# DeepRank/Deeprank-GNN

Hardware: AMD Instinct MI355X
Metric: interface-graphs/sec (fwd+bwd) GINet batch=64 per GPU (higher is better)
Workload: dtype f32; 1 GPU; GINet train step (topology + body fwd + FC head/MSE + bwd + grad all-reduce + Adam) on SYN graphs: 200 nodes, ~1000 directed edges, 32 node feats, 50->16 clusters (BASELINE.json configs[1]); graphs_per_gpu=64, global_batch=64, parallelism=dp1, mode=native, step_layout=auto

## Files before the change

### deeprank-gnn_amd/csrc/drgnn_step.h

```cpp
#ifndef DRGNN_STEP_H
#define DRGNN_STEP_H

#include "drgnn_net.h"

#ifndef DRGNN_SKIP
#define DRGNN_SKIP (-1)
#endif
#define PH(k) if (DRGNN_SKIP != (k))
#ifndef DRGNN_EXIT_AFTER
#define DRGNN_EXIT_AFTER (-1)
#endif
#define EXIT_AFTER(k)                                                                          \
    do {                                                                                       \
        if (DRGNN_EXIT_AFTER == (k)) {                                                         \
            float acc_ = 0.0f;                                                                 \
            if ((k) > 0) { FOR_TID(i_, (int)(s.end - scratch)) { acc_ += scratch[i_]; } }      \
            if (acc_ == 12345.678f) a.hf.pred[0] = acc_;                                       \
            return;                                                                            \
        }                                                                                      \
    } while (0)

struct StepArgs {
    drgnn_net_desc net;
    const float* x;
// ... 59 lines not shown
    X(mem1, capC, 1)                                                                           \
    X(a0, ((long)capC * DRGNN_H1 + 1) / 2, 1)                                                    \
    X(a1, ((long)capC * DRGNN_H2 + 1) / 2, 1)                                                    \
    X(u1, (long)(capN + 4) * hc1, 1)                                                           \
    X(z1, (long)capN * DRGNN_H1, 1)                                                            \
    X(dv0, capN, !gin)                                                                         \
    X(sc0, capN, !gin)                                                                         \
    X(xp, (long)(capC + 4) * STEP_XPLD, 1)                                                     \
    X(u2, (long)(capC + 4) * (DRGNN_H2 + 4), 1)                                                \
    X(z2, (long)(capC + 4) * (DRGNN_H2 + 4), 1)                                                \
    X(p2, (gin ? ((long)capC * DRGNN_H2 > (long)(capC + 4) * STEP_XPLD ? (long)capC * DRGNN_H2 : (long)(capC + 4) * STEP_XPLD) \
               : (long)(capC + 4) * (DRGNN_H2 + 4)), 1)                                        \
    X(dv1, capC, !gin)                                                                         \
    X(sc1, capC, !gin)                                                                         \
    X(hw2, (long)O * H, 1)                                                                     \
    X(hb2, O, 1)

HD int64_t step_scratch_words(int kind, int64_t F, int64_t capN, int64_t capE, int64_t capC, int64_t R,
                              int64_t H, int64_t O) {
    const int64_t hc1 = (kind == DRGNN_GINET) ? DRGNN_H1 : 2 * DRGNN_H1;
    const int64_t hc2 = (kind == DRGNN_GINET) ? DRGNN_H2 : 2 * DRGNN_H2;
    const int sg = (kind == DRGNN_SGAT) ? 1 : 0;
    const int gin = (kind == DRGNN_GINET) ? 1 : 0;
    const int64_t xld = step_pad16((int)F) + 4;
    int64_t w = 0;
#define X(name, words, cond) w += (cond) ? (((int64_t)(words) + 3) & ~(int64_t)3) : 0;
    STEP_CARVE_LIST(X)
#undef X
    return w + 16;
}

#define STEP_M_BAD 0
#define STEP_M_Y 1
#define STEP_M_WY 2
#define STEP_M_DENOM 3
#define STEP_WB_J 4

static inline bool step_burst_guaranteed(int kind, const float* x, int F, int capN, int capE, int capC, int H, int O) {
    if (H != ((kind == DRGNN_GINET) ? 128 : 64)) return false;
    return ((((uintptr_t)x) & 15) == 0) && (F % 4 == 0) && (F * DRGNN_H1 <= DRGNN_BCAP) && ((long)capN * F <= 16L * DRGNN_BCAP) &&
           (capN + 1 <= DRGNN_BCAP) && (capE <= 2 * DRGNN_BCAP) && (capC * DRGNN_H1 <= 4 * DRGNN_BCAP) &&
           O * H <= 2 * DRGNN_BCAP && H * 8 <= STEP_WB_J * DRGNN_BCAP;
}

#define STEP_CLS_N 200
#define STEP_CLS_E 1024
#define STEP_CLS_C 52

#ifndef DRGNN_EMU
#define STEP_PIN(x) asm volatile("" : "+v"(x))


template <bool RELU = false>
DEV void step_gemm_nn(int M, int NT, int K, const float* A, int lda, const float* Bt, int ldbt, float* C, int ldc,
                      int* dummy, const float* bias = nullptr, const float* nan_rows = nullptr, int wave_shift = 0) {
    const int wave = (__builtin_amdgcn_readfirstlane((int)(threadIdx.x >> 6)) - wave_shift) & (DRGNN_NWAVES - 1);
    const int lane = threadIdx.x & 63;
    const int lr = lane & 15, lq = lane >> 4;
    const int units = ((M + 15) >> 4) * NT;
    for (int u = wave; u < units; u += DRGNN_NWAVES) {
        const int ti = (NT == 1) ? u : (u >> 1), tj = (NT == 1) ? 0 : (u & 1);
        const float* ap = A + (ti * 16 + lr) * lda + 4 * lq;
        const float* bp = Bt + (tj * 16 + lr) * ldbt + 4 * lq;
        drgnn_f32x4 acc = {0.f, 0.f, 0.f, 0.f};
        for (int k0 = 0; k0 < K; k0 += 32) {
            const drgnn_f4 a0 = *(const drgnn_f4*)(ap + k0), b0 = *(const drgnn_f4*)(bp + k0);
            const bool two = k0 + 16 < K;
            drgnn_f4 a1 = a0, b1 = b0;
            if (two) { a1 = *(const drgnn_f4*)(ap + k0 + 16); b1 = *(const drgnn_f4*)(bp + k0 + 16); }
#pragma unroll
            for (int j = 0; j < 4; ++j) acc = __builtin_amdgcn_mfma_f32_16x16x4f32(a0[j], b0[j], acc, 0, 0, 0);
            if (two) {
#pragma unroll
                for (int j = 0; j < 4; ++j) acc = __builtin_amdgcn_mfma_f32_16x16x4f32(a1[j], b1[j], acc, 0, 0, 0);
            }
        }
#pragma unroll
        for (int r = 0; r < 4; ++r) {
            const int ci = ti * 16 + lq * 4 + r;
            float* p = (ci < M) ? C + ci * ldc + tj * 16 + lr : (float*)dummy + lane;
            float v = acc[r];
            if (bias) v += bias[tj * 16 + lr];
            if (nan_rows && ci < M && nan_rows[ci] == 0.0f) v = DRGNN_NAN;
            if (RELU) v = (v < 0.0f) ? 0.0f : v;
            *p = v;
        }
    }
}

template <int LD, class IdxT>
DEV void step_gather_rows(int n, const int* rp, const IdxT* col, const float* src, float* dst) {
    const int items = ((n * 16) + 63) & ~63;
    for (int item = threadIdx.x; item < items; item += DRGNN_NTHREADS) {
        const int i = item >> 4, sl = (item >> 2) & 3, c = (item & 3) * 4;
        float a0 = 0.f, a1 = 0.f, a2 = 0.f, a3 = 0.f;
        if (i < n) {
            const int lo = rp[i], hi = rp[i + 1];
            for (int k = lo + sl; k < hi; k += 4) {
                const drgnn_f4 v = *(const drgnn_f4*)(src + ROW24(col[k], LD) + c);
                a0 += v[0]; a1 += v[1]; a2 += v[2]; a3 += v[3];
            }
        }
        a0 += dpp_take<0x128>(a0); a1 += dpp_take<0x128>(a1); a2 += dpp_take<0x128>(a2); a3 += dpp_take<0x128>(a3);
        a0 += dpp_take<0x124>(a0); a1 += dpp_take<0x124>(a1); a2 += dpp_take<0x124>(a2); a3 += dpp_take<0x124>(a3);
        if (sl == 0 && i < n) *(drgnn_f4*)(dst + i * LD + c) = drgnn_f4{a0, a1, a2, a3};
    }
}

DEV void xchg_publish(unsigned long long* slot, uint32_t tag, float v);
template <int LDZ, bool SKIP0 = false>
DEV void step_pool_readout(int C1, const int* mp, const int* mem, const float* z, short* arg, const float* misc,
                           float* xr, float* g_readout, const int* rp = nullptr, unsigned long long* pub = nullptr,
                           uint32_t tag = 0u, int a1ld = 0) {
    int bad; memcpy(&bad, &misc[STEP_M_BAD], 4);
    const float inv = 1.0f / (float)(C1 > 0 ? C1 : 1);
    for (int t = threadIdx.x; t < DRGNN_H2 * 16; t += DRGNN_NTHREADS) {
        const int c = t >> 4, kk = t & 15;
        float acc = 0.0f;
        for (int k = kk; k < C1; k += 16) {
            float best = DRGNN_NEG_INF;
            int am = -1;
            const int plo = mp[k], phi = mp[k + 1];
            for (int p = plo; p < phi; p += 4) {
                int mm[4];
                float vv[4];
#pragma unroll
                for (int j = 0; j < 4; ++j) mm[j] = mem[(p + j < phi) ? p + j : phi - 1];
#pragma unroll
                for (int j = 0; j < 4; ++j) {
                    vv[j] = z[ROW24(mm[j], LDZ) + c];
                    if (SKIP0 && rp[mm[j] + 1] == rp[mm[j]]) vv[j] = DRGNN_NAN;
                }
#pragma unroll
                for (int j = 0; j < 4; ++j)
                    if (vv[j] > best) { best = vv[j]; am = mm[j]; }
            }
            if (am < 0) best = 0.0f;
            arg[a1ld ? c * a1ld + k : k * DRGNN_H2 + c] = (short)((best > 0.0f) ? am : -1);
            acc += best;
        }
        acc = lanes16_sum(acc) * inv;
        if (bad) acc = DRGNN_NAN;
        if (kk == 0) {
            if (pub) xchg_publish(pub + c, tag, acc);
            xr[c] = acc; out_store(&g_readout[c], acc);
        }
    }
}

DEV void xchg_publish(unsigned long long* slot, uint32_t tag, float v) {
    const unsigned long long w = ((unsigned long long)tag << 32) | (unsigned long long)__float_as_uint(v);
    __hip_atomic_store(slot, w, __ATOMIC_RELAXED, __HIP_MEMORY_SCOPE_AGENT);
}
DEV float xchg_wait(unsigned long long* slot, uint32_t tag, int32_t* fault) {
    const unsigned long long t0 = wall_clock64();
    for (;;) {
        const unsigned long long w = __hip_atomic_load(slot, __ATOMIC_RELAXED, __HIP_MEMORY_SCOPE_AGENT);
        if ((uint32_t)(w >> 32) == tag) return __uint_as_float((uint32_t)w);
        if (wall_clock64() - t0 > 30000000ull) { atomicOr(fault, DRGNN_FAULT_EXCHANGE); return DRGNN_NAN; }
        __builtin_amdgcn_s_sleep(1);
    }
}
DEV unsigned long long xchg_peek(const unsigned long long* slot) {
    return __hip_atomic_load(slot, __ATOMIC_RELAXED, __HIP_MEMORY_SCOPE_AGENT);
}
DEV float xchg_finish(unsigned long long* slot, unsigned long long w, uint32_t tag, int32_t* fault) {
    if ((uint32_t)(w >> 32) == tag) return __uint_as_float((uint32_t)w);
    return xchg_wait(slot, tag, fault);
}

template <int WJ> struct WBlockRegs { drgnn_f4 v[WJ * DRGNN_BSCALE]; };
template <int WJ> DEV void step_wblock_load(WBlockRegs<WJ>& wr, const HeadFused& hf, int br) {
    const bool vec = ((((uintptr_t)hf.w1) & 15) == 0);
#pragma unroll
    for (int j = 0; j < WJ * DRGNN_BSCALE; ++j) {
        const int t = threadIdx.x + j * DRGNN_NTHREADS;
        const int h = t >> 3, q = t & 7;
        drgnn_f4 v = {0.f, 0.f, 0.f, 0.f};
        if (h < hf.H) {
            const float* src = hf.w1 + (long)h * hf.R + br * DRGNN_H2 + 4 * q;
            if (vec) v = *(const drgnn_f4*)src;
            else { v[0] = src[0]; v[1] = src[1]; v[2] = src[2]; v[3] = src[3]; }
        }
        wr.v[j] = v;
    }
}
template <int WJ> DEV void step_wblock_store(const WBlockRegs<WJ>& wr, const HeadFused& hf, int br, float* wb) {
    (void)br;
#pragma unroll
    for (int j = 0; j < WJ * DRGNN_BSCALE; ++j) {
        const int t = threadIdx.x + j * DRGNN_NTHREADS;
        const int h = t >> 3, q = t & 7;
        if (h < hf.H) *(drgnn_f4*)(wb + h * STEP_WBLD + 4 * q) = wr.v[j];
    }
}

template <int HC, int WJ>
DEV void step_head_fc1_t(const HeadFused& hf, int g, int br, int nb, const float* wb, const WBlockRegs<WJ>& wo,
                         const float* b1, const float* xr, float* hid, unsigned long long* xg, uint32_t tag, uint32_t step,
                         uint32_t thresh, float keep_scale, int32_t* fault) {
    const int H = HC ? HC : hf.H;
    const int lane = threadIdx.x & 63;
    unsigned long long* const slot = xg + (long)(1 - br) * DRGNN_H2 + (lane & (DRGNN_H2 - 1));
    unsigned long long w0 = 0ull;
    if (nb > 1 && lane < DRGNN_H2) w0 = xchg_peek(slot);
    const int items = (H * 8 + 63) & ~63;
    drgnn_f4 xo = {0.f, 0.f, 0.f, 0.f};
    bool have_other = false;
    int j = 0;
    for (int t = threadIdx.x; t < items; t += DRGNN_NTHREADS, ++j) {
        const int h = t >> 3, q = t & 7;
        float acc = 0.0f;
        if (h < H) {
            const drgnn_f4 w = *(const drgnn_f4*)(wb + h * STEP_WBLD + 4 * q);
            const drgnn_f4 x = *(const drgnn_f4*)(xr + 4 * q);
            acc = fmaf(w[0], x[0], fmaf(w[1], x[1], fmaf(w[2], x[2], w[3] * x[3])));
        }
        acc = lanes8_sum(acc);
        float v = acc;
        if (nb > 1) {
            if (!have_other) {
                float pv = 0.0f;
                PH(7) { if (lane < DRGNN_H2) pv = xchg_finish(slot, w0, tag, fault); }
                const int src = (lane & 7) * 4;
                xo[0] = __shfl(pv, src, 64); xo[1] = __shfl(pv, src + 1, 64);
                xo[2] = __shfl(pv, src + 2, 64); xo[3] = __shfl(pv, src + 3, 64);
                have_other = true;
            }
            float other = 0.0f;
            if (h < H) {
                const drgnn_f4 w = wo.v[j < WJ * DRGNN_BSCALE ? j : 0];
                other = fmaf(w[0], xo[0], fmaf(w[1], xo[1], fmaf(w[2], xo[2], w[3] * xo[3])));
            }
            other = lanes8_sum(other);
            v = (br == 0) ? acc + other : other + acc;
        }
        if (q == 0 && h < H) {
            v += b1[h];
            v = v > 0.0f ? v : 0.0f;
            if (thresh) v = drgnn_keep(hf, step, g, H, h, thresh) ? v * keep_scale : 0.0f;
            hid[h] = v;
        }
    }
}
template <int WREF, bool ONLY, int WJ>
DEV void step_head_fc1(const HeadFused& hf, int g, int br, int nb, const float* wb, const WBlockRegs<WJ>& wo, const float* b1,
                       const float* xr, float* hid, unsigned long long* xg, uint32_t tag, uint32_t step,
                       uint32_t thresh, float keep_scale, int32_t* fault) {
    if (ONLY || hf.H == WREF) step_head_fc1_t<WREF, WJ>(hf, g, br, nb, wb, wo, b1, xr, hid, xg, tag, step, thresh, keep_scale, fault);
    else step_head_fc1_t<0, WJ>(hf, g, br, nb, wb, wo, b1, xr, hid, xg, tag, step, thresh, keep_scale, fault);
}

template <int HC, int OC>
DEV void step_head_loss_t(const HeadFused& hf, int g, int br, const float* hid, const float* w2, const float* b2,
                          const float* misc, float keep_scale, float* dhid, float* p_dhid, float* p_hw2,
                          float* p_hb2, float* p_loss) {
    const int H = HC ? HC : hf.H, O = OC ? OC : hf.O;
    if (__builtin_expect(!hf.train, 0)) {
        if (br == 0) {
            FOR_TID(o, O) {
                float acc = b2[o];
                for (int h = 0; h < H; ++h) acc = fmaf(hid[h], w2[o * H + h], acc);
                if (hf.sigmoid && hf.task != DRGNN_TASK_CLASS) acc = drgnn_sigmoid(acc);
                out_store(&hf.pred[(long)g * O + o], acc);
            }
        }
        return;
    }
    const bool ext = hf.task == DRGNN_TASK_GRAD;
    const bool sig = hf.sigmoid && hf.task != DRGNN_TASK_CLASS;
    const float denom = misc[STEP_M_DENOM], wy = misc[STEP_M_WY];
    if ((int)(threadIdx.x & ~63u) >= H && threadIdx.x >= 64) return;
    const int lane = threadIdx.x & 63;
    if (HC != 0 && HC <= 128 && OC == 1 && hf.task != DRGNN_TASK_CLASS) {
        constexpr int NH = (HC > 0) ? (HC + 63) / 64 : 1;
        float hv[NH], wv[NH];
#pragma unroll
        for (int j = 0; j < NH; ++j) { hv[j] = hid[lane + 64 * j]; wv[j] = w2[lane + 64 * j]; }
        const float bias = b2[0], yv = misc[STEP_M_Y];
        float acc = 0.0f;
#pragma unroll
        for (int j = 0; j < NH; ++j) acc = fmaf(hv[j], wv[j], acc);
        float out = lanes64_sum(acc) + bias;
        if (sig) out = drgnn_sigmoid(out);
        const float inv = 1.0f / (float)(hf.B * O);
        const float d = out - yv;
        const float dout = (ext ? yv : 2.0f * d * inv) * (sig ? out * (1.0f - out) : 1.0f);
        const int wv_id = (int)(threadIdx.x >> 6);
        float hme = hv[0], wme = wv[0];
#pragma unroll
        for (int j = 1; j < NH; ++j) { if (wv_id == j) { hme = hv[j]; wme = wv[j]; } }
        const int h = (int)threadIdx.x;
        const float dh = (hme != 0.0f) ? fmaf(dout, wme, 0.0f) * keep_scale : 0.0f;
        dhid[h] = dh;
        if (br == 0) {
            out_store(&p_hw2[h], dout * hme);
            out_store(&p_dhid[h], dh);
            if (threadIdx.x == 0) {
                out_store(&hf.pred[(long)g], out);
                out_store(&p_hb2[0], dout);
                out_store(&p_loss[0], ext ? 0.0f : (d * d * inv));
                out_store(&p_loss[1], 1.0f);
            }
        }
        return;
    }
    float my_out = 0.0f;
    for (int o = 0; o < O; ++o) {
        float acc = 0.0f;
        for (int h = lane; h < H; h += 64) acc = fmaf(hid[h], w2[o * H + h], acc);
        acc = lanes64_sum(acc) + b2[o];
        if (lane == o) my_out = acc;
    }
    if (sig) my_out = drgnn_sigmoid(my_out);
    float my_dout = 0.0f, loss, wsum = 1.0f;
    if (ext) {
        loss = 0.0f;
        my_dout = lane < O ? hf.y_reg[(long)g * O + lane] * (sig ? my_out * (1.0f - my_out) : 1.0f) : 0.0f;
    } else if (__builtin_expect(hf.task == DRGNN_TASK_REG, 1)) {
        const float inv = 1.0f / (float)(hf.B * O);
        const float d = my_out - misc[STEP_M_Y];
        loss = lanes64_sum(lane < O ? d * d * inv : 0.0f);
        my_dout = lane < O ? 2.0f * d * inv * (sig ? my_out * (1.0f - my_out) : 1.0f) : 0.0f;
    } else {
        const int yc = __builtin_amdgcn_readfirstlane(__float_as_int(misc[STEP_M_Y]));
        const float mx = lanes64_max(lane < O ? my_out : DRGNN_NEG_INF);
        const float se = lanes64_sum(lane < O ? expf(my_out - mx) : 0.0f);
        const float lse = logf(se) + mx;
        loss = wy * (lse - lane_get(my_out, yc)) / denom;
        my_dout = lane < O ? wy * (expf(my_out - lse) - (lane == yc ? 1.0f : 0.0f)) / denom : 0.0f;
        wsum = wy;
    }
    if (br == 0 && (int)threadIdx.x < O) {
        out_store(&hf.pred[(long)g * O + threadIdx.x], my_out);
        out_store(&p_hb2[threadIdx.x], my_dout);
    }
    if (br == 0 && threadIdx.x == 0) { out_store(&p_loss[0], loss); out_store(&p_loss[1], wsum); }
    for (int h0 = 0; h0 < H; h0 += DRGNN_NTHREADS) {
        const int h = h0 + (int)threadIdx.x;
        const bool ok = h < H;
        const float hv = ok ? hid[h] : 0.0f;
        float acc = 0.0f;
        for (int o = 0; o < O; ++o) {
            const float dout = lane_get(my_dout, o);
            if (ok) {
                acc = fmaf(dout, w2[o * H + h], acc);
                if (br == 0) out_store(&p_hw2[(long)o * H + h], dout * hv);
            }
        }
        if (ok) {
            const float dh = (hv != 0.0f) ? acc * keep_scale : 0.0f;
            dhid[h] = dh;
            if (br == 0) out_store(&p_dhid[h], dh);
        }
    }
}
template <int WREF, bool ONLY>
DEV void step_head_loss(const HeadFused& hf, int g, int br, const float* hid, const float* w2, const float* b2,
                        const float* misc, float keep_scale, float* dhid, float* p_dhid, float* p_hw2,
                        float* p_hb2, float* p_loss) {
    if (__builtin_expect(hf.H == WREF && hf.O == 1, 1))
        step_head_loss_t<WREF, 1>(hf, g, br, hid, w2, b2, misc, keep_scale, dhid, p_dhid, p_hw2, p_hb2, p_loss);
    else
        step_head_loss_t<0, 0>(hf, g, br, hid, w2, b2, misc, keep_scale, dhid, p_dhid, p_hw2, p_hb2, p_loss);
}
#endif

#endif
```

### deeprank-gnn_amd/csrc/drgnn_step3.h

```cpp
#ifndef DRGNN_STEP3_H
#define DRGNN_STEP3_H

#include "drgnn_step2.h"
#include <type_traits>

#ifndef DRGNN_EMU
struct Step3Scratch {
    float* misc; float* xr; float* hid; float* dhid; float* hb1; float* wb;
    float* w1t; float* w2t; float* w2n;
    int* hmp;
    int* rp1; int* cx1; int* cp1; int* rx1; int* mp1; int* mem1;
    short* a0; short* a1;
    float* G; float* z1;
    float* xp; float* u2; float* z2; float* p2;
    float* hw2; float* hb2;
    float* end; float* gp;
};
#define STEP3_Z2LD (DRGNN_H2 + 4)
#define STEP3_A1LD(capC) (((capC) + 1) & ~1)
#define STEP3_CARVE_LIST(X)                                                                    \
    X(misc, 128)                                                                               \
    X(xr, 2 * DRGNN_H2)                                                                        \
    X(hid, H)                                                                                  \
    X(dhid, H)                                                                                 \
    X(hb1, H)                                                                                  \
    X(wb, step_gp_words((int)H))                                                               \
    X(w1t, DRGNN_H1 * xld)                                                                     \
    X(w2t, DRGNN_H2 * STEP_XPLD)                                                               \
    X(w2n, DRGNN_H1 * (DRGNN_H2 + 4))                                                          \
    X(hmp, capC + 1)                                                                           \
    X(rp1, capC + 1)                                                                           \
    X(cx1, capE)                                                                               \
    X(cp1, capC + 1)                                                                           \
    X(rx1, capE)                                                                               \
    X(mp1, capC + 1)                                                                           \
    X(mem1, capC)                                                                              \
    X(a0, ((long)STEP3_A1LD(capC) * DRGNN_H1 + 1) / 2)                                         \
    X(a1, ((long)STEP3_A1LD(capC) * DRGNN_H2 + 1) / 2)                                         \
    X(G, (long)(capN + 4) * xld)                                                               \
    X(z1, (long)(capN + 4) * DRGNN_H1)                                                         \
    X(xp, (long)(capC + 4) * STEP_XPLD)                                                        \
    X(u2, (long)(capC + 4) * STEP_XPLD)                                                        \
    X(z2, (long)(capC + 4) * STEP3_Z2LD)                                                       \
    X(p2, (long)(capC + 4) * STEP_XPLD)                                                        \
    X(hw2, (long)O * H)                                                                        \
    X(hb2, O)
#endif

HD int64_t step3_scratch_words(int64_t F, int64_t capN, int64_t capE, int64_t capC, int64_t H, int64_t O) {
    const int64_t xld = step_pad16((int)F) + 4;
    int64_t w = 0;
#ifndef DRGNN_EMU
#define X(name, words) w += (((int64_t)(words) + 3) & ~(int64_t)3);
    STEP3_CARVE_LIST(X)
#undef X
#else
    (void)xld; (void)capN; (void)capE; (void)capC; (void)H; (void)O;
    w = (int64_t)1 << 40;
#endif
    return w + 16;
}

#ifndef DRGNN_EMU
template <int CLS>
DEV Step3Scratch step3_carve(float* base, int F, int capN, int capE, int capC, int H, int O) {
    const int xld = step_pad16(F) + 4;
    Step3Scratch s;
    int o = 0;
#define X(name, words)                                                                          \
    { int off = o; if (CLS == 0) { STEP_PIN(off); } s.name = (decltype(s.name))(base + off);    \
      o = off + (int)(((long)(words) + 3) & ~3L); }
    STEP3_CARVE_LIST(X)
#undef X
    s.end = base + o;
    s.gp = s.wb;
    return s;
}

DEV void step3_cluster_max(int nc, const int* hmp, const int* cid, const float* z, float* xp, short* a0, int a0ld) {
    FOR_TID(item, nc * DRGNN_H1) {
        const int q = item >> 4, c = item & 15;
        const int plo = hmp[q], phi = hmp[q + 1];
        const int j = cid[q];
        float best = DRGNN_NEG_INF;
        int arg = -1;
        for (int p = plo; p < phi; p += 4) {
            int mm[4];
            float vv[4];
#pragma unroll
            for (int t = 0; t < 4; ++t) mm[t] = (p + t < phi) ? p + t : phi - 1;
#pragma unroll
            for (int t = 0; t < 4; ++t) vv[t] = z[mm[t] * DRGNN_H1 + c];
#pragma unroll
            for (int t = 0; t < 4; ++t)
                if (vv[t] > best) { best = vv[t]; arg = mm[t]; }
        }
        if (arg < 0) best = 0.0f;
        xp[ROW24(j, STEP_XPLD) + c] = best;
        a0[c * a0ld + j] = (short)((best > 0.0f) ? arg : -1);
    }
}

template <int HC>
DEV void step3_dreadout_dw2(const float* wb, const float* dhid, const short* a1, int a1ld, int C1, const float* s2, float* z2,
                            float* g_dw2) {
    const float inv = 1.0f / (float)(C1 > 0 ? C1 : 1);
    for (int t = threadIdx.x; t < DRGNN_H2 * 32; t += DRGNN_NTHREADS) {
        const int c = t >> 5, q = t & 31;
        float acc = 0.0f;
#pragma unroll
        for (int h = q; h < HC; h += 32) acc = fmaf(dhid[h], wb[h * STEP_WBLD + c], acc);
        const float v = lanes32_sum(acc) * inv;
        const short* a1c = a1 + c * a1ld;
        for (int k = q; k < C1; k += 32) {
            const int r = a1c[k];
            if (r >= 0) z2[ROW24(r, STEP3_Z2LD) + c] = v;
        }
        const int sl = q & 7, f4 = q >> 3;
        drgnn_f4 sum = {0.f, 0.f, 0.f, 0.f};
        for (int k = sl; k < C1; k += 8) {
            const int r = a1c[k];
            if (r >= 0) {
                const drgnn_f4 row = *(const drgnn_f4*)(s2 + ROW24(r, STEP_XPLD) + 4 * f4);
                sum[0] += row[0]; sum[1] += row[1]; sum[2] += row[2]; sum[3] += row[3];
            }
        }
#pragma unroll
        for (int i = 0; i < 4; ++i) sum[i] = lanes8_sum(sum[i]);
        if (sl == 0) {
#pragma unroll
            for (int i = 0; i < 4; ++i) out_store(&g_dw2[(4 * f4 + i) * DRGNN_H2 + c], v * sum[i]);
        }
    }
}
template <int LD>
DEV void step3_gather_dxp(int n, const int* cp, const int* ridx, const float* src, float* dst) {
    const int items = ((n * 16) + 63) & ~63;
    for (int item = threadIdx.x; item < items; item += DRGNN_NTHREADS) {
        const int j = item >> 4, sl = (item >> 2) & 3, c = (item & 3) * 4;
        float a0 = 0.f, a1 = 0.f, a2 = 0.f, a3 = 0.f;
        if (j < n) {
            const int lo = cp[j], hi = cp[j + 1];
            for (int t = lo + sl; t < hi; t += 4) {
                const drgnn_f4 v = *(const drgnn_f4*)(src + ROW24(ridx[t], LD) + c);
                a0 += v[0]; a1 += v[1]; a2 += v[2]; a3 += v[3];
            }
        }
        a0 += dpp_take<0x128>(a0); a1 += dpp_take<0x128>(a1); a2 += dpp_take<0x128>(a2); a3 += dpp_take<0x128>(a3);
        a0 += dpp_take<0x124>(a0); a1 += dpp_take<0x124>(a1); a2 += dpp_take<0x124>(a2); a3 += dpp_take<0x124>(a3);
        if (sl == 0 && j < n) *(drgnn_f4*)(dst + j * LD + c) = drgnn_f4{a0, a1, a2, a3};
    }
}
template <int XF, bool SG = false>
DEV void step3_dw1_sparse(int C, const short* a0, int a0ld, const float* dxp, const float* G, float* g_dw1, int F,
                          const int* hord = nullptr, int gtf = 0) {
    constexpr int XLD = XF + 4, NSL = Dw1Shape<XF>::NSL;
    const int h = threadIdx.x >> 6, fc = (threadIdx.x & 63) / NSL, sl = threadIdx.x & (NSL - 1);
    const bool live = 4 * fc < XF;
    drgnn_f4 acc = {0.f, 0.f, 0.f, 0.f};
    for (int j = sl; j < C; j += 4 * NSL) {
        int arg[4];
        float d[4];
#pragma unroll
        for (int u = 0; u < 4; ++u) {
            const int jj = j + NSL * u;
            arg[u] = (jj < C && live) ? (int)a0[h * a0ld + jj] : -1;
            d[u] = (jj < C) ? dxp[jj * STEP_XPLD + h] : 0.0f;
        }
#pragma unroll
        for (int u = 0; u < 4; ++u) {
            if (arg[u] >= 0) {
                const drgnn_f4 g = !SG ? *(const drgnn_f4*)(G + ROW24(arg[u], XLD) + 4 * fc)
                                       : (4 * fc < gtf ? *(const drgnn_f4*)(G + (long)hord[arg[u]] * gtf + 4 * fc) : drgnn_f4{0.f, 0.f, 0.f, 0.f});
                acc[0] = fmaf(d[u], g[0], acc[0]); acc[1] = fmaf(d[u], g[1], acc[1]);
                acc[2] = fmaf(d[u], g[2], acc[2]); acc[3] = fmaf(d[u], g[3], acc[3]);
            }
        }
    }
#pragma unroll
    for (int i = 0; i < 4; ++i) acc[i] = step_slices_sum<NSL>(acc[i]);
    if (sl == 0) {
#pragma unroll
        for (int i = 0; i < 4; ++i)
            if (4 * fc + i < F) g_dw1[(4 * fc + i) * DRGNN_H1 + h] = acc[i];
    }
}

template <int XF>
DEV void step3_conv1_sg(int n, const float* sgl, int gtf, const int* hord, const float* w1t, float* z1, int* dummy) {
    constexpr int XLD = XF + 4;
    const int wave = __builtin_amdgcn_readfirstlane((int)(threadIdx.x >> 6)), lane = threadIdx.x & 63;
    const int lr = lane & 15, lq = lane >> 4;
    const int units = (n + 15) >> 4;
    for (int ti = wave; ti < units; ti += DRGNN_NWAVES) {
        const int prow = ti * 16 + lr;
        const int row = prow < n ? prow : n - 1;
        const float* ag = sgl + (long)hord[row] * gtf + 4 * lq;
        drgnn_f4 av[XF / 16];
#pragma unroll
        for (int k0 = 0; k0 < XF; k0 += 16)
            av[k0 / 16] = (k0 + 4 * lq < gtf) ? *(const drgnn_f4*)(ag + k0) : drgnn_f4{0.f, 0.f, 0.f, 0.f};
        const float* bp = w1t + lr * XLD + 4 * lq;
        drgnn_f32x4 acc = {0.f, 0.f, 0.f, 0.f};
#pragma unroll
        for (int k0 = 0; k0 < XF; k0 += 16) {
            const drgnn_f4 a = av[k0 / 16], b = *(const drgnn_f4*)(bp + k0);
#pragma unroll
            for (int j = 0; j < 4; ++j) acc = __builtin_amdgcn_mfma_f32_16x16x4f32(a[j], b[j], acc, 0, 0, 0);
        }
#pragma unroll
        for (int r = 0; r < 4; ++r) {
            const int ci = ti * 16 + lq * 4 + r;
            float* p = (ci < n) ? z1 + ci * DRGNN_H1 + lr : (float*)dummy + lane;
            const float v = acc[r];
            *p = (v < 0.0f) ? 0.0f : v;
        }
    }
}

template <int XF, bool GATHER, int CLS, bool TRAIN = true>
DEV void net_step3_graph(const StepArgs& a, const GraphDims& d_in, int g, int gi, int br, float* scratch, int capN, int capE,
                         int capC, bool late, int cnt_c, int cnt_e1, int cnt_c1) {
    static_assert(XF == 16 || XF == 32 || XF == 48 || XF == 64, "width-specialised kernels only");
    if (CLS == 1) { capN = STEP_CLS_N; capE = STEP_CLS_E; capC = STEP_CLS_C; }
    GraphDims d = d_in;
    const int bC = late ? imin(d.N, capC) : d.C, bE1 = late ? d.E : d.E1, bC1 = late ? imin(d.N, capC) : d.C1;
    const TopoView& tv = a.tv;
    const HeadFused& hf = a.hf;
    constexpr int nb = 2, R = 2 * DRGNN_H2, WREF = 128;
    constexpr int XLD = XF + 4, Z2LD = STEP3_Z2LD, W2NLD = DRGNN_H2 + 4;
    const int F = a.net.n_feat;
    const int O = hf.O;
    Step3Scratch s = step3_carve<CLS>(scratch, XF, capN, capE, capC, WREF, O);
    EXIT_AFTER(0);
    WBlockRegs<1> wreg, wother;
    int* const dummy = (int*)(s.misc + 64);
    const uint32_t done = (uint32_t)a.step2[0];
    const uint32_t tag = done + 1u;
    const drgnn_conv_params& c1 = a.net.conv1[br];
    const drgnn_conv_params& c2 = a.net.conv2[br];

    PHASE_MARK();
    const int TF = (F + 3) & ~3;
    const float* sgl = a.tiles + (long)d.n0 * TF;
    BurstX<4> bx;
    BurstRowMap<4> brow;
    BurstW<1> bw1, bw2;
    WaveStage wst;
    const int my_wave = __builtin_amdgcn_readfirstlane((int)(threadIdx.x >> 6));
    auto stage_job = [&](int burst, int w) -> StageJob {
        const int32_t* const* P = tv.p;
        StageJob j = {nullptr, 0, nullptr, 0};
        switch (burst * 16 + w) {
        case 16 + 0: j = StageJob{P[DRGNN_TI_HMP0] + d.rowbase, bC + 1, s.hmp, 0}; break;
        case 16 + 1: j = StageJob{P[DRGNN_TI_MEM1] + d.n0, bC, s.mem1, 0}; break;
        case 16 + 2: j = StageJob{P[DRGNN_TI_MPTR1] + d.rowbase, bC1 + 1, s.mp1, 0}; break;
        case 16 + 3: j = StageJob{hf.b1, WREF, s.hb1, 0}; break;
        case 16 + 4: j = stage_half(StageJob{hf.w2, O * WREF, s.hw2, 0}, 0); break;
        case 16 + 5: j = stage_half(StageJob{hf.w2, O * WREF, s.hw2, 0}, 1); break;
        case 16 + 6: j = StageJob{hf.b2, O, s.hb2, 0}; break;
        case 16 + 7: j = StageJob{P[DRGNN_TI_ROWPTR1] + d.rowbase, bC + 1, s.rp1, 0}; break;
        case 16 + 8: j = stage_half(StageJob{P[DRGNN_TI_COL1] + d.e0, bE1, s.cx1, 0}, 0); break;
        case 16 + 9: j = stage_half(StageJob{P[DRGNN_TI_COL1] + d.e0, bE1, s.cx1, 0}, 1); break;
        case 16 + 10: if (TRAIN) j = StageJob{P[DRGNN_TI_COLPTR1] + d.rowbase, bC + 1, s.cp1, 0}; break;
        case 16 + 11: if (TRAIN) j = stage_half(StageJob{P[DRGNN_TI_ROWIDX1] + d.e0, bE1, s.rx1, 0}, 0); break;
        case 16 + 12: if (TRAIN) j = stage_half(StageJob{P[DRGNN_TI_ROWIDX1] + d.e0, bE1, s.rx1, 0}, 1); break;
        default: break;
        }
        return j;
    };
    {
        const int32_t* const* P = tv.p;
        asm volatile("" :: "s"(P[DRGNN_TI_IHORD]), "s"(P[DRGNN_TI_HMP0]), "s"(P[DRGNN_TI_MEM1]), "s"(P[DRGNN_TI_MPTR1]));
        asm volatile("" :: "s"(P[DRGNN_TI_ROWPTR1]), "s"(P[DRGNN_TI_COL1]), "s"(P[DRGNN_TI_COLPTR1]), "s"(P[DRGNN_TI_ROWIDX1]));
    }
    int m_bad = 0, m_y = 0;
    float m_wy = 1.0f, m_denom = 1.0f;
    if (my_wave == 0) {
        m_bad = tv.p[DRGNN_TI_ERR][0] | tv.p[DRGNN_TI_GSTAT][gi] | tv.p[DRGNN_TI_GSTAT][(GATHER ? a.ws_graphs : a.n_graphs) + gi];
        if (!TRAIN) {
        } else if (__builtin_expect(hf.task != DRGNN_TASK_CLASS, 1)) {
            m_y = __builtin_nontemporal_load((const int*)hf.y_reg + gi);
        } else {
            m_y = (int)hf.y_cls[gi];
            m_wy = hf.class_w ? hf.class_w[m_y] : 1.0f;
            m_denom = (float)hf.B;
            if (hf.class_w && threadIdx.x < 64) {
                float part_sum = 0.0f;
                for (int q = threadIdx.x; q < hf.B; q += 64) part_sum += hf.class_w[hf.y_cls[GATHER ? a.gather_ids[q] : q]];
                m_denom = lanes64_sum(part_sum);
            }
            m_y = __builtin_amdgcn_readfirstlane(m_y);
            m_wy = __int_as_float(__builtin_amdgcn_readfirstlane(__float_as_int(m_wy)));
            m_bad = __builtin_amdgcn_readfirstlane(m_bad);
        }
    }
    burst_load_x(bx, sgl, d.N, TF);
    burst_load_rowmap(brow, bx, tv.p[DRGNN_TI_IHORD] + d.n0, d.N);
    burst_load_w(bw1, c1.w_nbr, c1.nbr_sk, c1.nbr_sh, F, DRGNN_H1);
    wstage_load(wst, stage_job(1, my_wave));
    burst_load_w(bw2, c2.w_nbr, c2.nbr_sk, c2.nbr_sh, DRGNN_H1, DRGNN_H2);
    step_wblock_load(wreg, hf, br);
    step_wblock_load(wother, hf, 1 - br);
    burst_store_x4_rows(bx, brow, s.G, XLD);
    burst_store_wt(bw1, s.w1t, XLD);
    wstage_store(wst);
    FOR_TID(e, (step_pad4(d.N) - d.N) * XLD) { s.G[d.N * XLD + e] = 0.0f; }
    if (XF > TF) {
        const int padg = XF - TF;
        FOR_TID(e, d.N * padg) { s.G[(e / padg) * XLD + TF + e % padg] = 0.0f; }
    }
    if (XF > F) {
        const int padc = XF - F;
        FOR_TID(e, DRGNN_H1 * padc) { s.w1t[(e / padc) * XLD + F + e % padc] = 0.0f; }
    }
    FOR_TID(i, 1) {
        ((int*)s.misc)[STEP_M_BAD] = m_bad;
        ((int*)s.misc)[STEP_M_Y] = m_y;
        s.misc[STEP_M_WY] = m_wy;
        s.misc[STEP_M_DENOM] = m_denom;
    }
    BARRIER();
    EXIT_AFTER(1);
    if (late) { d.C = WG_UNIFORM(cnt_c); d.E1 = WG_UNIFORM(cnt_e1); d.C1 = WG_UNIFORM(cnt_c1); }
    int bad_shape = 0;
    if (d.C > capC || d.E1 > d.E || d.C1 > capC) {
        d.C = imin(d.C, capC); d.E1 = imin(d.E1, d.E); d.C1 = imin(d.C1, capC);
        bad_shape = 1;
    }

    EXIT_AFTER(2);
    PH(2) step_gemm_nn<true>(d.N, 1, XF, s.G, XLD, s.w1t, XLD, s.z1, DRGNN_H1, dummy);
    burst_store_wt(bw2, s.w2t, STEP_XPLD);
    if (TRAIN) burst_store_w(bw2, s.w2n, W2NLD);
    step_wblock_store(wreg, hf, br, s.wb);
    FOR_TID(e, (step_pad4(d.C) - d.C) * STEP_XPLD) { s.xp[d.C * STEP_XPLD + e] = 0.0f; }
    if (bad_shape) { FOR_TID(i, 1) { ((int*)s.misc)[STEP_M_BAD] = 1; } }
    BARRIER();
    EXIT_AFTER(3);
    PH(3) step3_cluster_max(d.C, s.hmp, s.mem1, s.z1, s.xp, s.a0, STEP3_A1LD(capC));
    BARRIER();
    EXIT_AFTER(4);
    PH(4) step_gather_rows<STEP_XPLD, int>(d.C, s.rp1, s.cx1, s.xp, s.u2);
    FOR_TID(e, (step_pad4(d.C) - d.C) * STEP_XPLD) { s.u2[d.C * STEP_XPLD + e] = 0.0f; }
    BARRIER();
    EXIT_AFTER(5);
    PH(5) step_gemm_nn<true>(d.C, 2, DRGNN_H1, s.u2, STEP_XPLD, s.w2t, STEP_XPLD, s.z2, Z2LD, dummy);
    BARRIER();
    EXIT_AFTER(6);
    PH(6) step_pool_readout<Z2LD>(d.C1, s.mp1, s.mem1, s.z2, s.a1, s.misc, s.xr,
                                  const_cast<float*>(hf.readout) + (long)g * R + br * DRGNN_H2, nullptr,
                                  a.xchg + (long)g * nb * WREF + br * DRGNN_H2, tag, STEP3_A1LD(capC));
    BARRIER();
    EXIT_AFTER(8);

    const float keep_scale = (hf.p_drop > 0.0f) ? 1.0f / (1.0f - hf.p_drop) : 1.0f;
    const double pt = (double)hf.p_drop * 4294967296.0;
    const uint32_t thresh = (hf.p_drop > 0.0f) ? (uint32_t)(pt > 4294967295.0 ? 4294967295.0 : pt) : 0u;
    float* hp = hf.partials + (long)g * head_compact_floats(R, WREF, O);
    float* p_dhid = hp;
    float* p_hw2 = p_dhid + WREF;
    float* p_hb2 = p_hw2 + (long)O * WREF;
    float* p_loss = p_hb2 + O;
    if (TRAIN && g == 0 && br == 0) { FOR_TID(i, 1) { a.step2[1] = (int32_t)tag; } }
    if (TRAIN) { FOR_TID(item, step_pad4(d.C) * Z2LD) { s.z2[item] = 0.0f; } }
    PH(8) step_head_fc1<WREF, true>(hf, g, br, nb, s.wb, wother, s.hb1, s.xr, s.hid, a.xchg + (long)g * nb * WREF, tag, done,
                                    thresh, keep_scale, a.step2 + 2);
    BARRIER();
    EXIT_AFTER(9);
    if (!TRAIN) {
        FOR_TID(c, DRGNN_H2) {
            __hip_atomic_store(a.xchg + (long)g * nb * WREF + (1 - br) * DRGNN_H2 + c, 0ull, __ATOMIC_RELAXED, __HIP_MEMORY_SCOPE_AGENT);
        }
    }
    PH(9) step_head_loss<WREF, true>(hf, g, br, s.hid, s.hw2, s.hb2, s.misc, keep_scale, s.dhid, p_dhid, p_hw2, p_hb2, p_loss);
    if (!TRAIN) return;
    BARRIER();
    EXIT_AFTER(10);
    float* part_w = a.partials + ((long)g * nb + br) * a.n_partial;
    float* p_w1n = part_w;
    float* p_w2n = p_w1n + 2L * F * DRGNN_H1 + DRGNN_H1;
    PH(10) step3_dreadout_dw2<WREF>(s.wb, s.dhid, s.a1, STEP3_A1LD(capC), d.C1, s.u2, s.z2, p_w2n);
    BARRIER();
    EXIT_AFTER(11);

    PH(11) step_gemm_nn(d.C, 1, DRGNN_H2, s.z2, Z2LD, s.w2n, W2NLD, s.p2, STEP_XPLD, dummy);
    BARRIER();
    EXIT_AFTER(12);
    PH(13) step3_gather_dxp<STEP_XPLD>(d.C, s.cp1, s.rx1, s.p2, s.xp);
    BARRIER();
    EXIT_AFTER(14);
    PH(16) step3_dw1_sparse<XF>(d.C, s.a0, STEP3_A1LD(capC), s.xp, s.G, p_w1n, F);
}


struct Step3BScratch {
    float* misc; float* xr; float* hid; float* dhid; float* hb1; float* wb;
    float* w1t[2]; float* w2t[2]; float* w2n[2];
    int* hmp;
    int* rp1; int* cx1; int* cp1; int* rx1; int* mp1; int* mem1;
    short* a0[2]; short* a1[2];
    float* G; float* z1;
    float* xp; float* u2[2]; float* z2[2]; float* p2;
    float* hw2; float* hb2;
    int* hord;
    float* end; float* gp;
};
#define STEP3B_CARVE_LIST(X)                                                                   \
    X(misc, 128)                                                                               \
    X(xr, 2 * DRGNN_H2)                                                                        \
    X(hid, H)                                                                                  \
    X(dhid, H)                                                                                 \
    X(hb1, H)                                                                                  \
    X(wb, step_gp_words((int)H))                                                               \
    X(w1t[0], DRGNN_H1 * xld)                                                                  \
    X(w1t[1], DRGNN_H1 * xld)                                                                  \
    X(w2t[0], DRGNN_H2 * STEP_XPLD)                                                            \
    X(w2t[1], DRGNN_H2 * STEP_XPLD)                                                            \
    X(w2n[0], DRGNN_H1 * (DRGNN_H2 + 4))                                                       \
    X(w2n[1], DRGNN_H1 * (DRGNN_H2 + 4))                                                       \
    X(hmp, capC + 1)                                                                           \
    X(rp1, capC + 1)                                                                           \
    X(cx1, capE)                                                                               \
    X(cp1, capC + 1)                                                                           \
    X(rx1, capE)                                                                               \
    X(mp1, capC + 1)                                                                           \
    X(mem1, capC)                                                                              \
    X(a0[0], ((long)STEP3_A1LD(capC) * DRGNN_H1 + 1) / 2)                                      \
    X(a0[1], ((long)STEP3_A1LD(capC) * DRGNN_H1 + 1) / 2)                                      \
    X(a1[0], ((long)STEP3_A1LD(capC) * DRGNN_H2 + 1) / 2)                                      \
    X(a1[1], ((long)STEP3_A1LD(capC) * DRGNN_H2 + 1) / 2)                                      \
    X(G, sg ? 4 : (long)(capN + 4) * xld)                                                      \
    X(z1, (long)(capN + 4) * DRGNN_H1)                                                         \
    X(xp, (long)(capC + 4) * STEP_XPLD)                                                        \
    X(u2[0], (long)(capC + 4) * STEP_XPLD)                                                     \
    X(z2[0], (long)(capC + 4) * STEP3_Z2LD)                                                    \
    X(u2[1], (long)(capC + 4) * STEP_XPLD)       \
    X(z2[1], (long)(capC + 4) * STEP3_Z2LD)                                                    \
    X(p2, (long)(capC + 4) * STEP_XPLD)                                                        \
    X(hw2, (long)O * H)                                                                        \
    X(hb2, O)                                                                                  \
    X(hord, sg ? capN : 0)
#endif

HD int64_t step3b_scratch_words(int64_t F, int64_t capN, int64_t capE, int64_t capC, int64_t H, int64_t O, int sg = 0) {
    const int64_t xld = step_pad16((int)F) + 4;
    int64_t w = 0;
#ifndef DRGNN_EMU
#define X(name, words) w += (((int64_t)(words) + 3) & ~(int64_t)3);
    STEP3B_CARVE_LIST(X)
#undef X
#else
    (void)xld; (void)capN; (void)capE; (void)capC; (void)H; (void)O; (void)sg;
    w = (int64_t)1 << 40;
#endif
    return w + 16;
}

#define STEP3B_DUAL(XF, CLS, TRAIN) (((XF) == 32 || (XF) == 48) && (CLS) == 1)
HD int64_t step3b_dual_extra_words(int64_t capN, int64_t capC) {
    (void)capN;
    return 2 * ((((capC + 4) * STEP_XPLD) + 3) & ~(int64_t)3);
}

#ifndef DRGNN_EMU
#define STEP3D_NT (DRGNN_NTHREADS / 2)
#define STEP3D_NW (DRGNN_NWAVES / 2)
template <bool RELU>
DEV void step3d_gemm_nn(int vwave, int M, int NT, int K, const float* A, int lda, const float* Bt, int ldbt, float* C, int ldc,
                        int* dummy) {
    const int lane = threadIdx.x & 63;
    const int lr = lane & 15, lq = lane >> 4;
    const int units = ((M + 15) >> 4) * NT;
    for (int u = vwave; u < units; u += STEP3D_NW) {
        const int ti = (NT == 1) ? u : (u >> 1), tj = (NT == 1) ? 0 : (u & 1);
        const float* ap = A + (ti * 16 + lr) * lda + 4 * lq;
        const float* bp = Bt + (tj * 16 + lr) * ldbt + 4 * lq;
        drgnn_f32x4 acc = {0.f, 0.f, 0.f, 0.f};
        for (int k0 = 0; k0 < K; k0 += 32) {
            const drgnn_f4 a0 = *(const drgnn_f4*)(ap + k0), b0 = *(const drgnn_f4*)(bp + k0);
            const bool two = k0 + 16 < K;
            drgnn_f4 a1 = a0, b1 = b0;
            if (two) { a1 = *(const drgnn_f4*)(ap + k0 + 16); b1 = *(const drgnn_f4*)(bp + k0 + 16); }
#pragma unroll
            for (int j = 0; j < 4; ++j) acc = __builtin_amdgcn_mfma_f32_16x16x4f32(a0[j], b0[j], acc, 0, 0, 0);
            if (two) {
#pragma unroll
                for (int j = 0; j < 4; ++j) acc = __builtin_amdgcn_mfma_f32_16x16x4f32(a1[j], b1[j], acc, 0, 0, 0);
            }
        }
#pragma unroll
        for (int r = 0; r < 4; ++r) {
            const int ci = ti * 16 + lq * 4 + r;
            float* p = (ci < M) ? C + ci * ldc + tj * 16 + lr : (float*)dummy + lane;
            float v = acc[r];
            if (RELU) v = (v < 0.0f) ? 0.0f : v;
            *p = v;
        }
    }
}
DEV void step3d_cluster_max(int tid, int nc, const int* hmp, const int* cid, const float* z, float* xp, short* a0, int a0ld) {
    _Pragma("nounroll") for (int item = tid; item < nc * DRGNN_H1; item += STEP3D_NT) {
        const int q = item >> 4, c = item & 15;
        const int plo = hmp[q], phi = hmp[q + 1];
        const int j = cid[q];
        float best = DRGNN_NEG_INF;
        int arg = -1;
        for (int p = plo; p < phi; p += 4) {
            int mm[4];
            float vv[4];
#pragma unroll
            for (int t = 0; t < 4; ++t) mm[t] = (p + t < phi) ? p + t : phi - 1;
#pragma unroll
            for (int t = 0; t < 4; ++t) vv[t] = z[mm[t] * DRGNN_H1 + c];
#pragma unroll
            for (int t = 0; t < 4; ++t)
                if (vv[t] > best) { best = vv[t]; arg = mm[t]; }
        }
        if (arg < 0) best = 0.0f;
        xp[ROW24(j, STEP_XPLD) + c] = best;
        a0[c * a0ld + j] = (short)((best > 0.0f) ? arg : -1);
    }
}
template <int LD>
DEV void step3d_gather16(int tid, int n, const int* ptr, const int* idx, const float* src, float* dst) {
    const int items = ((n * 16) + 63) & ~63;
    for (int item = tid; item < items; item += STEP3D_NT) {
        const int i = item >> 4, sl = (item >> 2) & 3, c = (item & 3) * 4;
        float a0 = 0.f, a1 = 0.f, a2 = 0.f, a3 = 0.f;
        if (i < n) {
            const int lo = ptr[i], hi = ptr[i + 1];
            for (int k = lo + sl; k < hi; k += 4) {
                const drgnn_f4 v = *(const drgnn_f4*)(src + ROW24(idx[k], LD) + c);
                a0 += v[0]; a1 += v[1]; a2 += v[2]; a3 += v[3];
            }
        }
        a0 += dpp_take<0x128>(a0); a1 += dpp_take<0x128>(a1); a2 += dpp_take<0x128>(a2); a3 += dpp_take<0x128>(a3);
        a0 += dpp_take<0x124>(a0); a1 += dpp_take<0x124>(a1); a2 += dpp_take<0x124>(a2); a3 += dpp_take<0x124>(a3);
        if (sl == 0 && i < n) *(drgnn_f4*)(dst + i * LD + c) = drgnn_f4{a0, a1, a2, a3};
    }
}
template <int LDZ>
DEV void step3d_pool_readout(int tid, int C1, const int* mp, const int* mem, const float* z, short* arg, const float* misc,
                             float* xr, float* g_readout, int a1ld) {
    int bad; memcpy(&bad, &misc[STEP_M_BAD], 4);
// ... 329 lines not shown
```

Baseline: 3.761 million graphs/s.

## Overlap dW2 pooled-row sums with cross-block exchange wait in FC1

Moves the pooled s2 row-sum computation for dW2 out of the backward dreadout phase and runs it as 'meanwhile' work while waiting for the partner block's readout exchange in FC1. The sums are parked in the W2^T scratch area and consumed later. It also replaces the single-peek spin with a multi-in-flight polling chain of atomic loads across all lanes. The aim is to hide exchange latency behind useful work. In exchange it reuses scratch that must be dead at that point, and it adds register pressure from the held load queue.

```diff
diff --git a/deeprank-gnn_amd/csrc/drgnn_step.h b/deeprank-gnn_amd/csrc/drgnn_step.h
--- a/deeprank-gnn_amd/csrc/drgnn_step.h
+++ b/deeprank-gnn_amd/csrc/drgnn_step.h
@@ -235,6 +235,46 @@
     const unsigned long long w = ((unsigned long long)tag << 32) | (unsigned long long)__float_as_uint(v);
     __hip_atomic_store(slot, w, __ATOMIC_RELAXED, __HIP_MEMORY_SCOPE_AGENT);
 }
+#define XCHG_INFLIGHT 3
+#define XCHG_CHAIN 9
+struct XchgTail { unsigned long long q[XCHG_INFLIGHT]; };
+DEV void xchg_tail_init(XchgTail& t) {
+#pragma unroll
+    for (int i = 0; i < XCHG_INFLIGHT; ++i) t.q[i] = 0ull;
+}
+DEV void xchg_retire(const XchgTail& t) {
+#pragma unroll
+    for (int i = 0; i < XCHG_INFLIGHT; ++i) asm volatile("" :: "v"(t.q[i]));
+}
+#define XCHG_POLL(i)                                                                                \
+    {                                                                                              \
+        const unsigned long long w_ = q[i];                                                        \
+        const bool hit_ = pending && (uint32_t)(w_ >> 32) == tag;                                  \
+        v = hit_ ? __uint_as_float((uint32_t)w_) : v;                                              \
+        pending = pending && !hit_;                                                                \
+        q[i] = __hip_atomic_load(slot, __ATOMIC_RELAXED, __HIP_MEMORY_SCOPE_AGENT);                \
+        if (__builtin_amdgcn_ballot_w64(pending) == 0ull) return v;                                \
+    }
+template <int HAVE>
+DEV float xchg_spin(unsigned long long* slot, uint32_t tag, int32_t* fault, unsigned long long (&q)[XCHG_INFLIGHT]) {
+    const unsigned long long t0 = wall_clock64();
+#pragma unroll
+    for (int i = HAVE; i < XCHG_INFLIGHT; ++i) q[i] = __hip_atomic_load(slot, __ATOMIC_RELAXED, __HIP_MEMORY_SCOPE_AGENT);
+    float v = DRGNN_NAN;
+    bool pending = true;
+#pragma unroll
+    for (int n = 0; n < XCHG_CHAIN; ++n) XCHG_POLL(n % XCHG_INFLIGHT)
+    for (;;) {
+#pragma unroll
+        for (int i = 0; i < XCHG_INFLIGHT; ++i) XCHG_POLL(i)
+        if (wall_clock64() - t0 > 30000000ull) {
+            if (pending) atomicOr(fault, DRGNN_FAULT_EXCHANGE);
+            return v;
+        }
+        __builtin_amdgcn_s_sleep(1);
+    }
+}
+#undef XCHG_POLL
 DEV float xchg_wait(unsigned long long* slot, uint32_t tag, int32_t* fault) {
     const unsigned long long t0 = wall_clock64();
     for (;;) {
@@ -250,6 +290,9 @@
 DEV float xchg_finish(unsigned long long* slot, unsigned long long w, uint32_t tag, int32_t* fault) {
     if ((uint32_t)(w >> 32) == tag) return __uint_as_float((uint32_t)w);
     return xchg_wait(slot, tag, fault);
+}
+DEV float xchg_finish2(unsigned long long* slot, XchgTail& t, uint32_t tag, int32_t* fault) {
+    return xchg_spin<2>(slot, tag, fault, t.q);
 }
 
 template <int WJ> struct WBlockRegs { drgnn_f4 v[WJ * DRGNN_BSCALE]; };
@@ -278,15 +321,18 @@
     }
 }
 
-template <int HC, int WJ>
+struct StepNoWork { DEV void operator()() const {} };
+template <int HC, int WJ, bool PIPE, class Meanwhile>
 DEV void step_head_fc1_t(const HeadFused& hf, int g, int br, int nb, const float* wb, const WBlockRegs<WJ>& wo,
                          const float* b1, const float* xr, float* hid, unsigned long long* xg, uint32_t tag, uint32_t step,
-                         uint32_t thresh, float keep_scale, int32_t* fault) {
+                         uint32_t thresh, float keep_scale, int32_t* fault, XchgTail& xt, const Meanwhile& meanwhile) {
     const int H = HC ? HC : hf.H;
     const int lane = threadIdx.x & 63;
     unsigned long long* const slot = xg + (long)(1 - br) * DRGNN_H2 + (lane & (DRGNN_H2 - 1));
-    unsigned long long w0 = 0ull;
-    if (nb > 1 && lane < DRGNN_H2) w0 = xchg_peek(slot);
+    xchg_tail_init(xt);
+    if (nb > 1 && (PIPE || lane < DRGNN_H2)) xt.q[0] = xchg_peek(slot);
+    meanwhile();
+    if (nb > 1 && PIPE) xt.q[1] = xchg_peek(slot);
     const int items = (H * 8 + 63) & ~63;
     drgnn_f4 xo = {0.f, 0.f, 0.f, 0.f};
     bool have_other = false;
@@ -304,7 +350,10 @@
         if (nb > 1) {
             if (!have_other) {
                 float pv = 0.0f;
-                PH(7) { if (lane < DRGNN_H2) pv = xchg_finish(slot, w0, tag, fault); }
+                PH(7) {
+                    if (PIPE) pv = xchg_finish2(slot, xt, tag, fault);
+                    else if (lane < DRGNN_H2) pv = xchg_finish(slot, xt.q[0], tag, fault);
+                }
                 const int src = (lane & 7) * 4;
                 xo[0] = __shfl(pv, src, 64); xo[1] = __shfl(pv, src + 1, 64);
                 xo[2] = __shfl(pv, src + 2, 64); xo[3] = __shfl(pv, src + 3, 64);
@@ -326,12 +375,14 @@
         }
     }
 }
-template <int WREF, bool ONLY, int WJ>
+template <int WREF, bool ONLY, bool PIPE, int WJ, class Meanwhile = StepNoWork>
 DEV void step_head_fc1(const HeadFused& hf, int g, int br, int nb, const float* wb, const WBlockRegs<WJ>& wo, const float* b1,
                        const float* xr, float* hid, unsigned long long* xg, uint32_t tag, uint32_t step,
-                       uint32_t thresh, float keep_scale, int32_t* fault) {
-    if (ONLY || hf.H == WREF) step_head_fc1_t<WREF, WJ>(hf, g, br, nb, wb, wo, b1, xr, hid, xg, tag, step, thresh, keep_scale, fault);
-    else step_head_fc1_t<0, WJ>(hf, g, br, nb, wb, wo, b1, xr, hid, xg, tag, step, thresh, keep_scale, fault);
+                       uint32_t thresh, float keep_scale, int32_t* fault, XchgTail& xt,
+                       const Meanwhile& meanwhile = Meanwhile()) {
+    if (ONLY || hf.H == WREF)
+        step_head_fc1_t<WREF, WJ, PIPE>(hf, g, br, nb, wb, wo, b1, xr, hid, xg, tag, step, thresh, keep_scale, fault, xt, meanwhile);
+    else step_head_fc1_t<0, WJ, PIPE>(hf, g, br, nb, wb, wo, b1, xr, hid, xg, tag, step, thresh, keep_scale, fault, xt, meanwhile);
 }
 
 template <int HC, int OC>
diff --git a/deeprank-gnn_amd/csrc/drgnn_step3.h b/deeprank-gnn_amd/csrc/drgnn_step3.h
--- a/deeprank-gnn_amd/csrc/drgnn_step3.h
+++ b/deeprank-gnn_amd/csrc/drgnn_step3.h
@@ -101,12 +101,37 @@
     }
 }
 
-template <int HC>
+DEV drgnn_f4 step3_dw2_sum(const short* a1c, int C1, const float* s2, int sl, int f4) {
+    drgnn_f4 sum = {0.f, 0.f, 0.f, 0.f};
+    for (int k = sl; k < C1; k += 8) {
+        const int r = a1c[k];
+        if (r >= 0) {
+            const drgnn_f4 row = *(const drgnn_f4*)(s2 + ROW24(r, STEP_XPLD) + 4 * f4);
+            sum[0] += row[0]; sum[1] += row[1]; sum[2] += row[2]; sum[3] += row[3];
+        }
+    }
+#pragma unroll
+    for (int i = 0; i < 4; ++i) sum[i] = lanes8_sum(sum[i]);
+    return sum;
+}
+#define STEP3_DW2_SUM_WORDS (DRGNN_H2 * DRGNN_H1)
+DEV void step3_dw2_sums(const short* a1, int a1ld, int C1, const float* s2, float* sums) {
+    for (int t = threadIdx.x; t < DRGNN_H2 * 32; t += DRGNN_NTHREADS) {
+        const int c = t >> 5, q = t & 31;
+        const int sl = q & 7, f4 = q >> 3;
+        const drgnn_f4 sum = step3_dw2_sum(a1 + c * a1ld, C1, s2, sl, f4);
+        if (sl == 0) *(drgnn_f4*)(sums + c * DRGNN_H1 + 4 * f4) = sum;
+    }
+}
+template <int HC, bool PRE = false>
 DEV void step3_dreadout_dw2(const float* wb, const float* dhid, const short* a1, int a1ld, int C1, const float* s2, float* z2,
-                            float* g_dw2) {
+                            float* g_dw2, const float* sums = nullptr) {
     const float inv = 1.0f / (float)(C1 > 0 ? C1 : 1);
     for (int t = threadIdx.x; t < DRGNN_H2 * 32; t += DRGNN_NTHREADS) {
         const int c = t >> 5, q = t & 31;
+        const int sl = q & 7, f4 = q >> 3;
+        drgnn_f4 sum = {0.f, 0.f, 0.f, 0.f};
+        if (PRE && sl == 0) sum = *(const drgnn_f4*)(sums + c * DRGNN_H1 + 4 * f4);
         float acc = 0.0f;
 #pragma unroll
         for (int h = q; h < HC; h += 32) acc = fmaf(dhid[h], wb[h * STEP_WBLD + c], acc);
@@ -116,17 +141,7 @@
             const int r = a1c[k];
             if (r >= 0) z2[ROW24(r, STEP3_Z2LD) + c] = v;
         }
-        const int sl = q & 7, f4 = q >> 3;
-        drgnn_f4 sum = {0.f, 0.f, 0.f, 0.f};
-        for (int k = sl; k < C1; k += 8) {
-            const int r = a1c[k];
-            if (r >= 0) {
-                const drgnn_f4 row = *(const drgnn_f4*)(s2 + ROW24(r, STEP_XPLD) + 4 * f4);
-                sum[0] += row[0]; sum[1] += row[1]; sum[2] += row[2]; sum[3] += row[3];
-            }
-        }
-#pragma unroll
-        for (int i = 0; i < 4; ++i) sum[i] = lanes8_sum(sum[i]);
+        if (!PRE) sum = step3_dw2_sum(a1c, C1, s2, sl, f4);
         if (sl == 0) {
 #pragma unroll
             for (int i = 0; i < 4; ++i) out_store(&g_dw2[(4 * f4 + i) * DRGNN_H2 + c], v * sum[i]);
@@ -364,8 +379,16 @@
     float* p_loss = p_hb2 + O;
     if (TRAIN && g == 0 && br == 0) { FOR_TID(i, 1) { a.step2[1] = (int32_t)tag; } }
     if (TRAIN) { FOR_TID(item, step_pad4(d.C) * Z2LD) { s.z2[item] = 0.0f; } }
-    PH(8) step_head_fc1<WREF, true>(hf, g, br, nb, s.wb, wother, s.hb1, s.xr, s.hid, a.xchg + (long)g * nb * WREF, tag, done,
-                                    thresh, keep_scale, a.step2 + 2);
+    static_assert(STEP3_DW2_SUM_WORDS <= DRGNN_H2 * STEP_XPLD, "the parked sums must fit W2^T's area");
+    float* const dw2_sums = s.w2t;
+    const short* const a1 = s.a1;
+    const float* const s2 = s.u2;
+    const int a1ld = STEP3_A1LD(capC), C1 = d.C1;
+    auto meanwhile = [&]() { if (TRAIN) { PH(10) step3_dw2_sums(a1, a1ld, C1, s2, dw2_sums); } };
+    XchgTail xt;
+    xchg_tail_init(xt);
+    PH(8) step_head_fc1<WREF, true, TRAIN>(hf, g, br, nb, s.wb, wother, s.hb1, s.xr, s.hid, a.xchg + (long)g * nb * WREF, tag, done,
+                                    thresh, keep_scale, a.step2 + 2, xt, meanwhile);
     BARRIER();
     EXIT_AFTER(9);
     if (!TRAIN) {
@@ -380,7 +403,7 @@
     float* part_w = a.partials + ((long)g * nb + br) * a.n_partial;
     float* p_w1n = part_w;
     float* p_w2n = p_w1n + 2L * F * DRGNN_H1 + DRGNN_H1;
-    PH(10) step3_dreadout_dw2<WREF>(s.wb, s.dhid, s.a1, STEP3_A1LD(capC), d.C1, s.u2, s.z2, p_w2n);
+    PH(10) step3_dreadout_dw2<WREF, true>(s.wb, s.dhid, s.a1, STEP3_A1LD(capC), d.C1, s.u2, s.z2, p_w2n, dw2_sums);
     BARRIER();
     EXIT_AFTER(11);
 
@@ -391,6 +414,7 @@
     BARRIER();
     EXIT_AFTER(14);
     PH(16) step3_dw1_sparse<XF>(d.C, s.a0, STEP3_A1LD(capC), s.xp, s.G, p_w1n, F);
+    xchg_retire(xt);
 }
 
 
```

Result: no change. 3.795 million graphs/s (median of 6 runs) (+0.9%).
